# 86885974647565434342125458569795756674/torch.distributed.pipeline.sync.Pipe

Hardware: AMD Instinct MI355X
Metric: tokens/sec for 12-layer Transformer at PP=N (pipeline-parallel training) (higher is better)
Workload: dtype bf16

## Files before the change

### mipipe/csrc/kernels/attention.hip

```cpp
#include "common.h"
#include "kernels.h"

namespace mipipe {

namespace {

typedef __attribute__((ext_vector_type(4))) short s16x4;
typedef __attribute__((ext_vector_type(8))) short s16x8;
typedef __attribute__((address_space(3))) s16x4 lds_s16x4;

constexpr int kRows = 64;
constexpr int kThreads = 256;
constexpr float kLog2e = 1.4426950408889634f;

template <int D>
struct Img {
  static constexpr int kRowBytes = 2 * D;
  static constexpr int kChunks = D / 8;
  static constexpr int kBytes = kRows * kRowBytes;
  __device__ static __forceinline__ int f(int r) {
    if constexpr (kChunks >= 16) return (((r ^ (r >> 2)) & 1) << 1) | ((r & 2) << 1) | (r & 8);
    else if constexpr (kChunks == 8) return ((((r >> 1) ^ (r >> 2)) & 1) << 1) | ((r >> 1) & 4);
    else return (((r & 3) << 2) | ((r >> 2) & 3)) & (kChunks - 1);
  }
// ... 533 lines not shown
        ds[j][r] = pr * (dp - dl[r]);
      }
    }
    scratch_write(scr, ds, lane);
    __builtin_amdgcn_s_waitcnt(0xC07F);
    const bf16x8 s0 = scratch_frag(scr, 0, lane);
    const bf16x8 s1 = scratch_frag(scr, 1, lane);
#pragma unroll
    for (int t2 = 0; t2 < ND; ++t2) {
      dq[t2] = __builtin_amdgcn_mfma_f32_16x16x32_bf16(s0, frag_cols<D>(kimg, 16 * t2, 0, lane), dq[t2], 0, 0, 0);
      dq[t2] = __builtin_amdgcn_mfma_f32_16x16x32_bf16(s1, frag_cols<D>(kimg, 16 * t2, 1, lane), dq[t2], 0, 0, 0);
    }
  }
  bf16_t* dQ = reinterpret_cast<bf16_t*>(a.dq) + boff;
#pragma unroll
  for (int t2 = 0; t2 < ND; ++t2)
#pragma unroll
    for (int r = 0; r < 4; ++r)
      dQ[(int64_t)(qrow0 + r) * a.ld_qkv + 16 * t2 + (lane & 15)] = f2bf(dq[t2][r] * a.scale);
}

template <bool CAUSAL>
__global__ void __launch_bounds__(kThreads, 2) attn_dq_wide_kernel(AttnArgs a) {
  constexpr int D = 64, NS = 2, ND = 4, RB = 2;
  extern __shared__ __attribute__((aligned(16))) char smem[];
  char* kimg = smem;
  char* vimg = smem + Img<D>::kBytes;
  bf16_t* scr_all = reinterpret_cast<bf16_t*>(smem + 2 * Img<D>::kBytes);

  const int tid = threadIdx.x, lane = tid & 63, wave = tid >> 6;
  const int qt = CAUSAL ? (int)gridDim.x - 1 - (int)blockIdx.x : (int)blockIdx.x;
  const int bh = blockIdx.y;
  const int b = bh / a.H, h = bh % a.H;
  const int q0 = qt * kWideRows;
  const int wrow0 = q0 + wave * 32;
  const int64_t boff = (int64_t)b * a.sb_qkv + (int64_t)h * a.sh_qkv;
  const int64_t koff = (int64_t)b * a.sb_qkv + (int64_t)kv_head(a, h) * a.sh_qkv;
  const bf16_t* Q = reinterpret_cast<const bf16_t*>(a.q) + boff;
  const bf16_t* K = reinterpret_cast<const bf16_t*>(a.k) + koff;
  const bf16_t* V = reinterpret_cast<const bf16_t*>(a.v) + koff;
  const bf16_t* dO = reinterpret_cast<const bf16_t*>(a.dout) + (int64_t)b * a.sb_o + (int64_t)h * a.sh_o;

  bf16x8 qf[RB][NS], df[RB][NS];
  float lse2[RB][4], dl[RB][4];
  f32x4 dq[RB][ND];
#pragma unroll
  for (int rb = 0; rb < RB; ++rb) {
    const int myrow = wrow0 + 16 * rb + (lane & 15);
#pragma unroll
    for (int s = 0; s < NS; ++s) {
      qf[rb][s] = frag_global(Q + (int64_t)myrow * a.ld_qkv, s, lane);
      df[rb][s] = frag_global(dO + (int64_t)myrow * a.ld_o, s, lane);
    }
    const int qrow0 = wrow0 + 16 * rb + 4 * (lane >> 4);
#pragma unroll
    for (int r = 0; r < 4; ++r) {
      lse2[rb][r] = a.lse[(int64_t)bh * a.S + qrow0 + r] * kLog2e;
      dl[rb][r] = a.delta[(int64_t)bh * a.S + qrow0 + r];
    }
#pragma unroll
    for (int t = 0; t < ND; ++t) dq[rb][t] = f32x4{0.f, 0.f, 0.f, 0.f};
  }
  const float sl2 = a.scale * kLog2e;
  const float pscale = a.p > 0.f ? 1.f / (1.f - a.p) : 1.f;
  const int ntiles = CAUSAL ? (q0 + kWideRows) / kRows : a.S / kRows;

  TileRegs kr, vr;
  load_tile<D>(K, a.ld_qkv, tid, kr);
  load_tile<D>(V, a.ld_qkv, tid, vr);
  for (int t = 0; t < ntiles; ++t) {
    const int k0 = t * kRows;
    __syncthreads();
    store_tile<D>(kimg, tid, kr);
    store_tile<D>(vimg, tid, vr);
    __syncthreads();
    if (t + 1 < ntiles) {
      load_tile<D>(K + (int64_t)(k0 + kRows) * a.ld_qkv, a.ld_qkv, tid, kr);
      load_tile<D>(V + (int64_t)(k0 + kRows) * a.ld_qkv, a.ld_qkv, tid, vr);
    }
    if (CAUSAL && k0 > wrow0 + 31) continue;
    const bool diag = CAUSAL && k0 + kRows - 1 > wrow0;

    f32x4 sacc[RB][4], pacc[RB][4];
#pragma unroll
    for (int rb = 0; rb < RB; ++rb)
#pragma unroll
      for (int j = 0; j < 4; ++j) sacc[rb][j] = pacc[rb][j] = f32x4{0.f, 0.f, 0.f, 0.f};
#pragma unroll
    for (int s = 0; s < NS; ++s)
#pragma unroll
      for (int j = 0; j < 4; ++j) {
        const bf16x8 kfr = frag_rows<D>(kimg, 16 * j, s, lane);
        const bf16x8 vfr = frag_rows<D>(vimg, 16 * j, s, lane);
#pragma unroll
        for (int rb = 0; rb < RB; ++rb) {
          sacc[rb][j] = __builtin_amdgcn_mfma_f32_16x16x32_bf16(qf[rb][s], kfr, sacc[rb][j], 0, 0, 0);
          pacc[rb][j] = __builtin_amdgcn_mfma_f32_16x16x32_bf16(df[rb][s], vfr, pacc[rb][j], 0, 0, 0);
        }
      }
#pragma unroll
    for (int rb = 0; rb < RB; ++rb) {
      const int qrow0 = wrow0 + 16 * rb + 4 * (lane >> 4);
      float ds[4][4];
#pragma unroll
      for (int j = 0; j < 4; ++j) {
        const int key = k0 + 16 * j + (lane & 15);
        uint32_t w[4] = {0xFFFFFFFFu, 0xFFFFFFFFu, 0xFFFFFFFFu, 0xFFFFFFFFu};
        if (a.p > 0.f) {
          const uint4 mw = attn_mask_words(a, bh, qrow0 >> 2, key);
          w[0] = mw.x; w[1] = mw.y; w[2] = mw.z; w[3] = mw.w;
        }
#pragma unroll
        for (int r = 0; r < 4; ++r) {
          float pr = __builtin_amdgcn_exp2f(sacc[rb][j][r] * sl2 - lse2[rb][r]);
          if (diag && key > qrow0 + r) pr = 0.f;
          float dp = pacc[rb][j][r];
          if (a.p > 0.f) dp = w[r] >= a.threshold ? dp * pscale : 0.f;
          ds[j][r] = pr * (dp - dl[rb][r]);
        }
      }
      scratch_write(scr_all + (wave * RB + rb) * 16 * kScrStride, ds, lane);
    }
    __builtin_amdgcn_s_waitcnt(0xC07F);
    bf16x8 sf[RB][2];
#pragma unroll
    for (int rb = 0; rb < RB; ++rb) {
      const bf16_t* scr = scr_all + (wave * RB + rb) * 16 * kScrStride;
      sf[rb][0] = scratch_frag(scr, 0, lane);
      sf[rb][1] = scratch_frag(scr, 1, lane);
    }
#pragma unroll
    for (int t2 = 0; t2 < ND; ++t2)
#pragma unroll
      for (int s = 0; s < 2; ++s) {
        const bf16x8 kc = frag_cols<D>(kimg, 16 * t2, s, lane);
#pragma unroll
        for (int rb = 0; rb < RB; ++rb)
          dq[rb][t2] = __builtin_amdgcn_mfma_f32_16x16x32_bf16(sf[rb][s], kc, dq[rb][t2], 0, 0, 0);
      }
  }
  bf16_t* dQ = reinterpret_cast<bf16_t*>(a.dq) + boff;
#pragma unroll
  for (int rb = 0; rb < RB; ++rb) {
    const int qrow0 = wrow0 + 16 * rb + 4 * (lane >> 4);
#pragma unroll
    for (int t2 = 0; t2 < ND; ++t2)
#pragma unroll
      for (int r = 0; r < 4; ++r)
        dQ[(int64_t)(qrow0 + r) * a.ld_qkv + 16 * t2 + (lane & 15)] = f2bf(dq[rb][t2][r] * a.scale);
  }
}

template <int D, bool CAUSAL>
__global__ void __launch_bounds__(kThreads, D >= 128 ? 1 : 2) attn_dkdv_kernel(AttnArgs a) {
  extern __shared__ __attribute__((aligned(16))) char smem[];
  char* qimg = smem;
  char* dimg = smem + Img<D>::kBytes;
  bf16_t* scr_all = reinterpret_cast<bf16_t*>(smem + 2 * Img<D>::kBytes);
  float* stats = reinterpret_cast<float*>(smem + 2 * Img<D>::kBytes + 4 * 16 * kScrStride * 2);

  const int tid = threadIdx.x, lane = tid & 63, wave = tid >> 6;
  const int kt = blockIdx.x, bh = blockIdx.y;
  const int b = bh / a.H, h = bh % a.H;
  const int k0 = kt * kRows;
  bf16_t* scr = scr_all + wave * 16 * kScrStride;
  const int64_t boff = (int64_t)b * a.sb_qkv + (int64_t)h * a.sh_qkv;
  const int64_t koff = (int64_t)b * a.sb_qkv + (int64_t)kv_head(a, h) * a.sh_qkv;
  const bf16_t* Q = reinterpret_cast<const bf16_t*>(a.q) + boff;
  const bf16_t* K = reinterpret_cast<const bf16_t*>(a.k) + koff;
  const bf16_t* V = reinterpret_cast<const bf16_t*>(a.v) + koff;
  const bf16_t* dO = reinterpret_cast<const bf16_t*>(a.dout) + (int64_t)b * a.sb_o + (int64_t)h * a.sh_o;

  constexpr int NS = D / 32, ND = D / 16;
  bf16x8 kf[NS], vf[NS];
  const int mykey = k0 + wave * 16 + (lane & 15);
#pragma unroll
  for (int s = 0; s < NS; ++s) {
    kf[s] = frag_global(K + (int64_t)mykey * a.ld_qkv, s, lane);
    vf[s] = frag_global(V + (int64_t)mykey * a.ld_qkv, s, lane);
  }
  const int key0 = k0 + wave * 16 + 4 * (lane >> 4);
  f32x4 dk[ND], dv[ND];
#pragma unroll
  for (int t = 0; t < ND; ++t) dk[t] = dv[t] = f32x4{0.f, 0.f, 0.f, 0.f};
  const float sl2 = a.scale * kLog2e;
  const float pscale = a.p > 0.f ? 1.f / (1.f - a.p) : 1.f;
  const int first = CAUSAL ? kt : 0;
  const int nq = a.S / kRows;

  constexpr bool PF = D <= 128;
  TileRegs qr, dr;
  if constexpr (PF) {
    load_tile<D>(Q + (int64_t)first * kRows * a.ld_qkv, a.ld_qkv, tid, qr);
    load_tile<D>(dO + (int64_t)first * kRows * a.ld_o, a.ld_o, tid, dr);
  }
  for (int t = first; t < nq; ++t) {
    const int q0 = t * kRows;
    __syncthreads();
    if constexpr (PF) {
      store_tile<D>(qimg, tid, qr);
      store_tile<D>(dimg, tid, dr);
    } else {
      stage_tile<D>(Q + (int64_t)q0 * a.ld_qkv, a.ld_qkv, qimg, tid);
      stage_tile<D>(dO + (int64_t)q0 * a.ld_o, a.ld_o, dimg, tid);
    }
    if (tid < 64) {
      stats[tid] = a.lse[(int64_t)bh * a.S + q0 + tid] * kLog2e;
      stats[64 + tid] = a.delta[(int64_t)bh * a.S + q0 + tid];
    }
    __syncthreads();
    if constexpr (PF) if (t + 1 < nq) {
      load_tile<D>(Q + (int64_t)(q0 + kRows) * a.ld_qkv, a.ld_qkv, tid, qr);
      load_tile<D>(dO + (int64_t)(q0 + kRows) * a.ld_o, a.ld_o, tid, dr);
    }
    f32x4 sacc[4], pacc[4];
#pragma unroll
    for (int j = 0; j < 4; ++j) sacc[j] = pacc[j] = f32x4{0.f, 0.f, 0.f, 0.f};
#pragma unroll
    for (int s = 0; s < NS; ++s)
#pragma unroll
      for (int j = 0; j < 4; ++j) {
        sacc[j] = __builtin_amdgcn_mfma_f32_16x16x32_bf16(kf[s], frag_rows<D>(qimg, 16 * j, s, lane), sacc[j], 0, 0, 0);
        pacc[j] = __builtin_amdgcn_mfma_f32_16x16x32_bf16(vf[s], frag_rows<D>(dimg, 16 * j, s, lane), pacc[j], 0, 0, 0);
      }
    float pd[4][4], ds[4][4];
#pragma unroll
    for (int j = 0; j < 4; ++j) {
      const int ql = 16 * j + (lane & 15);
      const int q = q0 + ql;
      const float l2 = stats[ql], dl = stats[64 + ql];
      uint32_t kw0 = 0xFFFFFFFFu, kw1 = 0xFFFFFFFFu, kw2 = 0xFFFFFFFFu, kw3 = 0xFFFFFFFFu;
      if (a.p > 0.f) {
        const int t = lane & 3;
        const uint4 mine = attn_mask_words(a, bh, q >> 2, key0 + t);
        auto word = [&](int i) { return i == 0 ? mine.x : (i == 1 ? mine.y : (i == 2 ? mine.z : mine.w)); };
#pragma unroll
        for (int k = 0; k < 4; ++k) {
          const int src = (lane & ~3) | ((t + k) & 3);
          const uint32_t got = (uint32_t)__shfl((int)word((t - k) & 3), src, 64);
          const int r = (t + k) & 3;
          kw0 = r == 0 ? got : kw0;
          kw1 = r == 1 ? got : kw1;
          kw2 = r == 2 ? got : kw2;
          kw3 = r == 3 ? got : kw3;
        }
      }
#pragma unroll
      for (int r = 0; r < 4; ++r) {
        const int key = key0 + r;
        float pr = __builtin_amdgcn_exp2f(sacc[j][r] * sl2 - l2);
        if (CAUSAL && key > q) pr = 0.f;
        float dp = pacc[j][r];
        float pdrop = pr;
        if (a.p > 0.f) {
          const uint32_t w = r == 0 ? kw0 : (r == 1 ? kw1 : (r == 2 ? kw2 : kw3));
          const bool keep = w >= a.threshold;
          pdrop = keep ? pr * pscale : 0.f;
          dp = keep ? dp * pscale : 0.f;
        }
        pd[j][r] = pdrop;
        ds[j][r] = pr * (dp - dl);
      }
    }
    scratch_write(scr, pd, lane);
    __builtin_amdgcn_s_waitcnt(0xC07F);
    bf16x8 f0 = scratch_frag(scr, 0, lane);
    bf16x8 f1 = scratch_frag(scr, 1, lane);
#pragma unroll
    for (int t2 = 0; t2 < ND; ++t2) {
      dv[t2] = __builtin_amdgcn_mfma_f32_16x16x32_bf16(f0, frag_cols<D>(dimg, 16 * t2, 0, lane), dv[t2], 0, 0, 0);
      dv[t2] = __builtin_amdgcn_mfma_f32_16x16x32_bf16(f1, frag_cols<D>(dimg, 16 * t2, 1, lane), dv[t2], 0, 0, 0);
    }
    __builtin_amdgcn_s_waitcnt(0xC07F);
    scratch_write(scr, ds, lane);
    __builtin_amdgcn_s_waitcnt(0xC07F);
    f0 = scratch_frag(scr, 0, lane);
    f1 = scratch_frag(scr, 1, lane);
#pragma unroll
    for (int t2 = 0; t2 < ND; ++t2) {
      dk[t2] = __builtin_amdgcn_mfma_f32_16x16x32_bf16(f0, frag_cols<D>(qimg, 16 * t2, 0, lane), dk[t2], 0, 0, 0);
      dk[t2] = __builtin_amdgcn_mfma_f32_16x16x32_bf16(f1, frag_cols<D>(qimg, 16 * t2, 1, lane), dk[t2], 0, 0, 0);
    }
  }
  const DkvDst dst = dkv_dst<0>(blockIdx.y);
  bf16_t* dK = dst.dk;
  bf16_t* dV = dst.dv;
#pragma unroll
  for (int t2 = 0; t2 < ND; ++t2)
#pragma unroll
    for (int r = 0; r < 4; ++r) {
      const int64_t o = (int64_t)(key0 + r) * dst.ld + 16 * t2 + (lane & 15);
      dK[o] = f2bf(dk[t2][r] * a.scale);
      dV[o] = f2bf(dv[t2][r]);
    }
}

namespace shortseq {

constexpr int S = 128;
constexpr int kThreads = 512;
constexpr int kChunk = 64;
constexpr int kChunkImg = S * kChunk * 2;
constexpr int kSqImg = S * S * 2;
constexpr int kStageBytes = 3 * kChunkImg;
constexpr int kPOff = 4 * kChunkImg;
constexpr int kDsOff = kPOff + kSqImg;
constexpr int kSmem = kDsOff + kSqImg;
constexpr int kFwdPOff = 2 * kChunkImg;
constexpr int kFwdSmem = kFwdPOff + kSqImg;

__device__ __forceinline__ int coff(int r, int c16) { return Img<64>::off(r, c16); }
__device__ __forceinline__ int soff(int r, int c16) { return Img<128>::off(r, c16); }

__device__ __forceinline__ void load_chunk(const bf16_t* __restrict__ base, int64_t ld, int d0, int tid, uint4& v0,
                                           uint4& v1) {
  const int r = tid >> 3, c = tid & 7;
  v0 = *reinterpret_cast<const uint4*>(base + (int64_t)r * ld + d0 + 8 * c);
  v1 = *reinterpret_cast<const uint4*>(base + (int64_t)(r + 64) * ld + d0 + 8 * c);
}
__device__ __forceinline__ void store_chunk(char* img, int tid, const uint4& v0, const uint4& v1) {
  const int r = tid >> 3, c = tid & 7;
  *reinterpret_cast<uint4*>(img + coff(r, c)) = v0;
  *reinterpret_cast<uint4*>(img + coff(r + 64, c)) = v1;
}

__device__ __forceinline__ bf16x8 crow(const char* img, int rb, int s, int lane) {
  return *reinterpret_cast<const bf16x8*>(img + coff(rb + (lane & 15), 4 * s + (lane >> 4)));
}
__device__ __forceinline__ bf16x8 ccol(const char* img, int db, int s, int lane) {
  const int g = lane >> 4, q = (lane & 15) >> 2, p = lane & 3;
  const int r0 = 32 * s + 8 * g + q;
  const int c8 = (db >> 2) + p;
  const int o0 = coff(r0, c8 >> 1) + 8 * (c8 & 1);
  const int o1 = coff(r0 + 4, c8 >> 1) + 8 * (c8 & 1);
  const s16x4 lo = __builtin_amdgcn_ds_read_tr16_b64_v4i16((lds_s16x4*)(img + o0));
  const s16x4 hi = __builtin_amdgcn_ds_read_tr16_b64_v4i16((lds_s16x4*)(img + o1));
  return __builtin_bit_cast(bf16x8, __builtin_shufflevector(lo, hi, 0, 1, 2, 3, 4, 5, 6, 7));
}
__device__ __forceinline__ bf16x8 srow(const char* img, int rb, int s, int lane) {
  return *reinterpret_cast<const bf16x8*>(img + soff(rb + (lane & 15), 4 * s + (lane >> 4)));
}
__device__ __forceinline__ bf16x8 scol(const char* img, int ib, int s, int lane) {
  const int g = lane >> 4, q = (lane & 15) >> 2, p = lane & 3;
  const int r0 = 32 * s + 8 * g + q;
  const int c8 = (ib >> 2) + p;
  const int o0 = soff(r0, c8 >> 1) + 8 * (c8 & 1);
  const int o1 = soff(r0 + 4, c8 >> 1) + 8 * (c8 & 1);
  const s16x4 lo = __builtin_amdgcn_ds_read_tr16_b64_v4i16((lds_s16x4*)(img + o0));
  const s16x4 hi = __builtin_amdgcn_ds_read_tr16_b64_v4i16((lds_s16x4*)(img + o1));
  return __builtin_bit_cast(bf16x8, __builtin_shufflevector(lo, hi, 0, 1, 2, 3, 4, 5, 6, 7));
}

template <int D, bool CAUSAL>
__global__ void __launch_bounds__(kThreads, 1) attn_bwd_s128_kernel(AttnArgs a) {
  extern __shared__ __attribute__((aligned(16))) char smem[];
  const int tid = threadIdx.x, lane = tid & 63, wave = __builtin_amdgcn_readfirstlane(tid >> 6);
  const int bh = blockIdx.x;
  const int b = bh / a.H, h = bh % a.H;
  const int64_t boff = (int64_t)b * a.sb_qkv + (int64_t)h * a.sh_qkv;
  const int64_t koff = (int64_t)b * a.sb_qkv + (int64_t)kv_head(a, h) * a.sh_qkv;
  const bf16_t* Q = reinterpret_cast<const bf16_t*>(a.q) + boff;
  const bf16_t* K = reinterpret_cast<const bf16_t*>(a.k) + koff;
  const bf16_t* V = reinterpret_cast<const bf16_t*>(a.v) + koff;
  const bf16_t* dO = reinterpret_cast<const bf16_t*>(a.dout) + (int64_t)b * a.sb_o + (int64_t)h * a.sh_o;
  constexpr int NC = D / kChunk;

  f32x4 sacc[8], pacc[8];
#pragma unroll
  for (int j = 0; j < 8; ++j) sacc[j] = pacc[j] = f32x4{0.f, 0.f, 0.f, 0.f};
  const int myrow = wave * 16 + (lane & 15);
  const bf16_t* qrow = Q + (int64_t)myrow * a.ld_qkv;
  const bf16_t* drow = dO + (int64_t)myrow * a.ld_o;

  uint4 k0, k1, v0, v1;
  load_chunk(K, a.ld_qkv, 0, tid, k0, k1);
  load_chunk(V, a.ld_qkv, 0, tid, v0, v1);
  store_chunk(smem, tid, k0, k1);
  store_chunk(smem + kChunkImg, tid, v0, v1);
  __syncthreads();
#pragma unroll 1
  for (int c = 0; c < NC; ++c) {
    const char* kimg = smem + (c & 1) * 2 * kChunkImg;
    const char* vimg = kimg + kChunkImg;
    if (c + 1 < NC) {
      load_chunk(K, a.ld_qkv, (c + 1) * kChunk, tid, k0, k1);
      load_chunk(V, a.ld_qkv, (c + 1) * kChunk, tid, v0, v1);
    }
    bf16x8 qf[2], df[2];
#pragma unroll
    for (int s2 = 0; s2 < 2; ++s2) {
      qf[s2] = frag_global(qrow + c * kChunk, s2, lane);
      df[s2] = frag_global(drow + c * kChunk, s2, lane);
    }
#pragma unroll
    for (int s2 = 0; s2 < 2; ++s2)
#pragma unroll
      for (int j = 0; j < 8; ++j) {
        sacc[j] = __builtin_amdgcn_mfma_f32_16x16x32_bf16(qf[s2], crow(kimg, 16 * j, s2, lane), sacc[j], 0, 0, 0);
        pacc[j] = __builtin_amdgcn_mfma_f32_16x16x32_bf16(df[s2], crow(vimg, 16 * j, s2, lane), pacc[j], 0, 0, 0);
      }
    if (c + 1 < NC) {
      char* nimg = smem + ((c + 1) & 1) * 2 * kChunkImg;
      store_chunk(nimg, tid, k0, k1);
      store_chunk(nimg + kChunkImg, tid, v0, v1);
    }
    __syncthreads();
  }

  const int qrow0 = wave * 16 + 4 * (lane >> 4);
  const float sl2 = a.scale * kLog2e;
  const float pscale = a.p > 0.f ? 1.f / (1.f - a.p) : 1.f;
  float lse2[4];
#pragma unroll
  for (int r = 0; r < 4; ++r) lse2[r] = a.lse[(int64_t)bh * S + qrow0 + r] * kLog2e;
  float dsum[4] = {0.f, 0.f, 0.f, 0.f};
#pragma unroll
  for (int j = 0; j < 8; ++j) {
    const int key = 16 * j + (lane & 15);
    uint32_t w[4] = {0xFFFFFFFFu, 0xFFFFFFFFu, 0xFFFFFFFFu, 0xFFFFFFFFu};
    if (a.p > 0.f) {
      const uint4 mw = attn_mask_words(a, bh, qrow0 >> 2, key);
      w[0] = mw.x; w[1] = mw.y; w[2] = mw.z; w[3] = mw.w;
    }
#pragma unroll
    for (int r = 0; r < 4; ++r) {
      float pr = __builtin_amdgcn_exp2f(sacc[j][r] * sl2 - lse2[r]);
      if (CAUSAL && key > qrow0 + r) pr = 0.f;
      float dp = pacc[j][r];
      float pd = pr;
      if (a.p > 0.f) {
        const bool keep = w[r] >= a.threshold;
        dp = keep ? dp * pscale : 0.f;
        pd = keep ? pr * pscale : 0.f;
      }
      sacc[j][r] = pr;
      pacc[j][r] = dp;
      dsum[r] += pr * dp;
      *reinterpret_cast<bf16_t*>(smem + kPOff + soff(qrow0 + r, key >> 3) + 2 * (key & 7)) = f2bf(pd);
    }
  }
  float delta[4];
#pragma unroll
  for (int r = 0; r < 4; ++r) delta[r] = row_reduce_sum16(dsum[r]);
#pragma unroll
  for (int j = 0; j < 8; ++j) {
    const int key = 16 * j + (lane & 15);
#pragma unroll
    for (int r = 0; r < 4; ++r) {
      const float ds = sacc[j][r] * (pacc[j][r] - delta[r]);
      *reinterpret_cast<bf16_t*>(smem + kDsOff + soff(qrow0 + r, key >> 3) + 2 * (key & 7)) = f2bf(ds);
    }
  }

  const char* pimg = smem + kPOff;
  const char* dsimg = smem + kDsOff;
  char* kimg = smem;
  char* qimg = smem + kChunkImg;
  char* dimg = smem + 2 * kChunkImg;
  const int r0 = wave * 16;
  uint4 a0, a1, b0, b1, e0, e1;
  load_chunk(K, a.ld_qkv, 0, tid, a0, a1);
  load_chunk(Q, a.ld_qkv, 0, tid, b0, b1);
  load_chunk(dO, a.ld_o, 0, tid, e0, e1);
#pragma unroll 1
  for (int c = 0; c < NC; ++c) {
    const int d0 = c * kChunk;
    __syncthreads();
    store_chunk(kimg, tid, a0, a1);
    store_chunk(qimg, tid, b0, b1);
    store_chunk(dimg, tid, e0, e1);
    __syncthreads();
    if (c + 1 < NC) {
      load_chunk(K, a.ld_qkv, d0 + kChunk, tid, a0, a1);
      load_chunk(Q, a.ld_qkv, d0 + kChunk, tid, b0, b1);
      load_chunk(dO, a.ld_o, d0 + kChunk, tid, e0, e1);
    }
    f32x4 dq[4], dk[4], dv[4];
#pragma unroll
    for (int t = 0; t < 4; ++t) dq[t] = dk[t] = dv[t] = f32x4{0.f, 0.f, 0.f, 0.f};
#pragma unroll
    for (int ks = 0; ks < 4; ++ks) {
      const bf16x8 a_dq = srow(dsimg, r0, ks, lane);
      const bf16x8 a_dk = scol(dsimg, r0, ks, lane);
      const bf16x8 a_dv = scol(pimg, r0, ks, lane);
#pragma unroll
      for (int t = 0; t < 4; ++t) {
        dq[t] = __builtin_amdgcn_mfma_f32_16x16x32_bf16(a_dq, ccol(kimg, 16 * t, ks, lane), dq[t], 0, 0, 0);
        dk[t] = __builtin_amdgcn_mfma_f32_16x16x32_bf16(a_dk, ccol(qimg, 16 * t, ks, lane), dk[t], 0, 0, 0);
        dv[t] = __builtin_amdgcn_mfma_f32_16x16x32_bf16(a_dv, ccol(dimg, 16 * t, ks, lane), dv[t], 0, 0, 0);
      }
    }
    const int orow = r0 + 4 * (lane >> 4);
    __syncthreads();
#pragma unroll
    for (int t = 0; t < 4; ++t) {
      const int col = 16 * t + (lane & 15);
#pragma unroll
      for (int r = 0; r < 4; ++r) {
        const int at = coff(orow + r, col >> 3) + 2 * (col & 7);
        *reinterpret_cast<bf16_t*>(kimg + at) = f2bf(dq[t][r] * a.scale);
        *reinterpret_cast<bf16_t*>(qimg + at) = f2bf(dk[t][r] * a.scale);
        *reinterpret_cast<bf16_t*>(dimg + at) = f2bf(dv[t][r]);
      }
    }
    __syncthreads();
    {
      const int r = tid >> 3, cc = tid & 7;
      const DkvDst dst = dkv_dst<0>(blockIdx.x);
      bf16_t* dK = dst.dk;
      bf16_t* dV = dst.dv;
      bf16_t* dQ = dq_dst<0>(blockIdx.x);
#pragma unroll
      for (int h2 = 0; h2 < 2; ++h2) {
        const int row = r + 64 * h2;
        const int off = coff(row, cc);
        const int64_t g = (int64_t)row * a.ld_qkv + d0 + 8 * cc;
        const int64_t gk = (int64_t)row * dst.ld + d0 + 8 * cc;
        *reinterpret_cast<uint4*>(dQ + g) = *reinterpret_cast<const uint4*>(kimg + off);
        *reinterpret_cast<uint4*>(dK + gk) = *reinterpret_cast<const uint4*>(qimg + off);
        *reinterpret_cast<uint4*>(dV + gk) = *reinterpret_cast<const uint4*>(dimg + off);
      }
    }
  }
}

template <int D, bool CAUSAL>
__global__ void __launch_bounds__(kThreads, 2) attn_fwd_s128_kernel(AttnArgs a) {
  extern __shared__ __attribute__((aligned(16))) char smem[];
  const int tid = threadIdx.x, lane = tid & 63, wave = __builtin_amdgcn_readfirstlane(tid >> 6);
  const int bh = blockIdx.x;
  const int b = bh / a.H, h = bh % a.H;
  const int64_t boff = (int64_t)b * a.sb_qkv + (int64_t)h * a.sh_qkv;
  const int64_t koff = (int64_t)b * a.sb_qkv + (int64_t)kv_head(a, h) * a.sh_qkv;
  const bf16_t* Q = reinterpret_cast<const bf16_t*>(a.q) + boff;
  const bf16_t* K = reinterpret_cast<const bf16_t*>(a.k) + koff;
  const bf16_t* V = reinterpret_cast<const bf16_t*>(a.v) + koff;
  constexpr int NC = D / kChunk;

  f32x4 sacc[8];
#pragma unroll
  for (int j = 0; j < 8; ++j) sacc[j] = f32x4{0.f, 0.f, 0.f, 0.f};
  const bf16_t* qrow = Q + (int64_t)(wave * 16 + (lane & 15)) * a.ld_qkv;

  uint4 k0, k1;
  load_chunk(K, a.ld_qkv, 0, tid, k0, k1);
  store_chunk(smem, tid, k0, k1);
  __syncthreads();
#pragma unroll 1
  for (int c = 0; c < NC; ++c) {
    const char* kimg = smem + (c & 1) * kChunkImg;
    if (c + 1 < NC) load_chunk(K, a.ld_qkv, (c + 1) * kChunk, tid, k0, k1);
    bf16x8 qf[2];
#pragma unroll
    for (int s2 = 0; s2 < 2; ++s2) qf[s2] = frag_global(qrow + c * kChunk, s2, lane);
#pragma unroll
    for (int s2 = 0; s2 < 2; ++s2)
#pragma unroll
      for (int j = 0; j < 8; ++j)
        sacc[j] = __builtin_amdgcn_mfma_f32_16x16x32_bf16(qf[s2], crow(kimg, 16 * j, s2, lane), sacc[j], 0, 0, 0);
    if (c + 1 < NC) store_chunk(smem + ((c + 1) & 1) * kChunkImg, tid, k0, k1);
    __syncthreads();
  }

  const int qrow0 = wave * 16 + 4 * (lane >> 4);
  const float sl2 = a.scale * kLog2e;
  const float pscale = a.p > 0.f ? 1.f / (1.f - a.p) : 1.f;
  float mx[4] = {-INFINITY, -INFINITY, -INFINITY, -INFINITY};
#pragma unroll
  for (int j = 0; j < 8; ++j) {
    const int key = 16 * j + (lane & 15);
#pragma unroll
    for (int r = 0; r < 4; ++r) {
      float x = sacc[j][r] * sl2;
      if (CAUSAL && key > qrow0 + r) x = -INFINITY;
      sacc[j][r] = x;
      mx[r] = fmaxf(mx[r], x);
    }
  }
#pragma unroll
  for (int r = 0; r < 4; ++r) mx[r] = row_reduce_max16(mx[r]);
  float sum[4] = {0.f, 0.f, 0.f, 0.f};
#pragma unroll
  for (int j = 0; j < 8; ++j)
#pragma unroll
    for (int r = 0; r < 4; ++r) {
      const float e = __builtin_amdgcn_exp2f(sacc[j][r] - mx[r]);
      sacc[j][r] = e;
      sum[r] += e;
    }
  float inv[4];
#pragma unroll
  for (int r = 0; r < 4; ++r) {
    sum[r] = row_reduce_sum16(sum[r]);
    inv[r] = 1.f / sum[r];
  }
  char* pimg = smem + kFwdPOff;
#pragma unroll
  for (int j = 0; j < 8; ++j) {
    const int key = 16 * j + (lane & 15);
    uint32_t w[4] = {0xFFFFFFFFu, 0xFFFFFFFFu, 0xFFFFFFFFu, 0xFFFFFFFFu};
    if (a.p > 0.f) {
      const uint4 mw = attn_mask_words(a, bh, qrow0 >> 2, key);
      w[0] = mw.x; w[1] = mw.y; w[2] = mw.z; w[3] = mw.w;
    }
#pragma unroll
    for (int r = 0; r < 4; ++r) {
      float pv = sacc[j][r] * inv[r];
      if (a.p > 0.f) pv = w[r] >= a.threshold ? pv * pscale : 0.f;
      *reinterpret_cast<bf16_t*>(pimg + soff(qrow0 + r, key >> 3) + 2 * (key & 7)) = f2bf(pv);
    }
  }
  if ((lane & 15) == 0) {
#pragma unroll
    for (int r = 0; r < 4; ++r) a.lse[(int64_t)bh * S + qrow0 + r] = (mx[r] + log2f(sum[r])) / kLog2e;
  }

  bf16_t* O = reinterpret_cast<bf16_t*>(a.o) + (int64_t)b * a.sb_o + (int64_t)h * a.sh_o;
  uint4 v0, v1;
  load_chunk(V, a.ld_qkv, 0, tid, v0, v1);
  store_chunk(smem, tid, v0, v1);
  __syncthreads();
  const int r0 = wave * 16;
#pragma unroll 1
  for (int c = 0; c < NC; ++c) {
    const char* vimg = smem + (c & 1) * kChunkImg;
    if (c + 1 < NC) load_chunk(V, a.ld_qkv, (c + 1) * kChunk, tid, v0, v1);
    f32x4 o[4];
#pragma unroll
    for (int t = 0; t < 4; ++t) o[t] = f32x4{0.f, 0.f, 0.f, 0.f};
#pragma unroll
    for (int ks = 0; ks < 4; ++ks) {
      const bf16x8 ap = srow(pimg, r0, ks, lane);
#pragma unroll
      for (int t = 0; t < 4; ++t)
        o[t] = __builtin_amdgcn_mfma_f32_16x16x32_bf16(ap, ccol(vimg, 16 * t, ks, lane), o[t], 0, 0, 0);
    }
    const int orow = r0 + 4 * (lane >> 4);
#pragma unroll
    for (int t = 0; t < 4; ++t)
#pragma unroll
      for (int r = 0; r < 4; ++r)
        O[(int64_t)(orow + r) * a.ld_o + c * kChunk + 16 * t + (lane & 15)] = f2bf(o[t][r]);
    if (c + 1 < NC) store_chunk(smem + ((c + 1) & 1) * kChunkImg, tid, v0, v1);
    __syncthreads();
  }
}

}

template <int D>
size_t fwd_smem() { return 2 * Img<D>::kBytes + 4 * 16 * kScrStride * 2; }
template <int D>
size_t dkdv_smem() { return fwd_smem<D>() + 128 * sizeof(float); }

int g_attn_fused_bwd = 1;
const int g_attn_wide = [] {
  const char* e = getenv("MIPIPE_ATTN_WIDE");
  return e == nullptr ? 1 : atoi(e);
}();

template <typename Kern>
void set_smem(Kern k, size_t bytes) {
  hipFuncSetAttribute(reinterpret_cast<const void*>(k), hipFuncAttributeMaxDynamicSharedMemorySize, (int)bytes);
}

template <int D, bool CAUSAL>
void run_fwd(const AttnArgs& a, hipStream_t s) {
  if (a.S == shortseq::S && g_attn_fused_bwd) {
    static bool once_s = false;
    if (!once_s) {
      set_smem(shortseq::attn_fwd_s128_kernel<D, CAUSAL>, shortseq::kFwdSmem);
      once_s = true;
    }
    hipLaunchKernelGGL((shortseq::attn_fwd_s128_kernel<D, CAUSAL>), dim3(a.B * a.H), dim3(shortseq::kThreads),
                       shortseq::kFwdSmem, s, a);
    return;
  }
  if (D == 64 && a.S % kWideRows == 0 && g_attn_wide) {
    static bool once_w = false;
    if (!once_w) { set_smem(attn_fwd_wide_kernel<CAUSAL>, wide_fwd_smem()); once_w = true; }
    hipLaunchKernelGGL((attn_fwd_wide_kernel<CAUSAL>), dim3(a.S / kWideRows, a.B * a.H), dim3(kThreads),
                       wide_fwd_smem(), s, a);
    return;
  }
  const size_t sm = fwd_smem<D>();
  static bool once = false;
  if (!once) { set_smem(attn_fwd_kernel<D, CAUSAL>, sm); once = true; }
  hipLaunchKernelGGL((attn_fwd_kernel<D, CAUSAL>), dim3(a.S / kRows, a.B * a.H), dim3(kThreads), sm, s, a);
}

template <int D, bool CAUSAL>
void run_bwd(const AttnArgs& a, hipStream_t s) {
  const size_t sm = fwd_smem<D>(), sm2 = dkdv_smem<D>();
  static bool once = false;
  if (!once) {
    set_smem(attn_dq_kernel<D, CAUSAL>, sm);
    set_smem(attn_dkdv_kernel<D, CAUSAL>, sm2);
    once = true;
  }
  if (a.S == shortseq::S && g_attn_fused_bwd) {
    static bool once_s = false;
    if (!once_s) {
      set_smem(shortseq::attn_bwd_s128_kernel<D, CAUSAL>, shortseq::kSmem);
      once_s = true;
    }
    hipLaunchKernelGGL((shortseq::attn_bwd_s128_kernel<D, CAUSAL>), dim3(a.B * a.H), dim3(shortseq::kThreads),
                       shortseq::kSmem, s, a);
    return;
  }
  const int64_t rows = (int64_t)a.B * a.S * a.H;
  hipLaunchKernelGGL(attn_delta_kernel, dim3((unsigned)((rows + 3) / 4)), dim3(256), 0, s, a, D);
  hipLaunchKernelGGL((attn_dkdv_kernel<D, CAUSAL>), dim3(a.S / kRows, a.B * a.H), dim3(kThreads), sm2, s, a);
  if (D == 64 && a.S % kWideRows == 0 && g_attn_wide) {
    static bool once_w = false;
    if (!once_w) { set_smem(attn_dq_wide_kernel<CAUSAL>, wide_fwd_smem()); once_w = true; }
    hipLaunchKernelGGL((attn_dq_wide_kernel<CAUSAL>), dim3(a.S / kWideRows, a.B * a.H), dim3(kThreads),
                       wide_fwd_smem(), s, a);
    return;
  }
  hipLaunchKernelGGL((attn_dq_kernel<D, CAUSAL>), dim3(a.S / kRows, a.B * a.H), dim3(kThreads), sm, s, a);
}

}

void attention_set_fused_bwd(int on) { g_attn_fused_bwd = on; }

bool attention_supported(int S, int D) { return S > 0 && S % kRows == 0 && (D == 64 || D == 128 || D == 256); }

void attention_fwd(const AttnArgs& ai, hipStream_t s) {
  AttnArgs a = attn_resolved(ai);
  a.threshold = dropout_threshold(a.p);
  if (a.causal) {
    if (a.D == 64) run_fwd<64, true>(a, s);
    else if (a.D == 128) run_fwd<128, true>(a, s);
    else run_fwd<256, true>(a, s);
  } else {
    if (a.D == 64) run_fwd<64, false>(a, s);
    else if (a.D == 128) run_fwd<128, false>(a, s);
    else run_fwd<256, false>(a, s);
  }
}

void attention_bwd(const AttnArgs& ai, hipStream_t s) {
  AttnArgs a = attn_resolved(ai);
  a.threshold = dropout_threshold(a.p);
  if (a.causal) {
    if (a.D == 64) run_bwd<64, true>(a, s);
    else if (a.D == 128) run_bwd<128, true>(a, s);
    else run_bwd<256, true>(a, s);
  } else {
    if (a.D == 64) run_bwd<64, false>(a, s);
    else if (a.D == 128) run_bwd<128, false>(a, s);
    else run_bwd<256, false>(a, s);
  }
}

}
```

Before: 147,500.

## Keep K resident in LDS and Q/dO fragments in registers for short-seq attention

In the fused S=128 backward kernel, all K chunks now stay resident in LDS and the Q/dO fragments loaded for the score pass are held in registers. The gradient pass reuses them instead of reloading K, Q and dO from global memory, and loads are issued two chunks ahead. The forward kernel prefetches the next Q fragment and the first V chunk during the score loop, and stages the O tile through LDS so global stores are coalesced 16-byte writes. The cost is more registers and LDS, with the full 160KB of LDS used at D=256, which may reduce occupancy.

```diff
diff --git a/mipipe/csrc/kernels/attention.hip b/mipipe/csrc/kernels/attention.hip
--- a/mipipe/csrc/kernels/attention.hip
+++ b/mipipe/csrc/kernels/attention.hip
@@ -859,10 +859,12 @@
 constexpr int kChunk = 64;
 constexpr int kChunkImg = S * kChunk * 2;
 constexpr int kSqImg = S * S * 2;
-constexpr int kStageBytes = 3 * kChunkImg;
-constexpr int kPOff = 4 * kChunkImg;
-constexpr int kDsOff = kPOff + kSqImg;
-constexpr int kSmem = kDsOff + kSqImg;
+constexpr int kBwdVOff = 0;
+constexpr int kBwdPOff = 2 * kChunkImg;
+constexpr int kBwdDsOff = kBwdPOff + kSqImg;
+constexpr int kBwdKOff = kBwdDsOff + kSqImg;
+template <int D> constexpr int bwd_smem() { return kBwdKOff + (D / kChunk) * kChunkImg; }
+static_assert(bwd_smem<256>() == 160 * 1024, "D = 256 uses exactly one CU's LDS");
 constexpr int kFwdPOff = 2 * kChunkImg;
 constexpr int kFwdSmem = kFwdPOff + kSqImg;
 
@@ -892,6 +894,18 @@
   const int o1 = coff(r0 + 4, c8 >> 1) + 8 * (c8 & 1);
   const s16x4 lo = __builtin_amdgcn_ds_read_tr16_b64_v4i16((lds_s16x4*)(img + o0));
   const s16x4 hi = __builtin_amdgcn_ds_read_tr16_b64_v4i16((lds_s16x4*)(img + o1));
+  return __builtin_bit_cast(bf16x8, __builtin_shufflevector(lo, hi, 0, 1, 2, 3, 4, 5, 6, 7));
+}
+__device__ __forceinline__ void ccol_off(int db, int lane, int& o0, int& o1) {
+  const int g = lane >> 4, q = (lane & 15) >> 2, p = lane & 3;
+  const int r0 = 8 * g + q;
+  const int c8 = (db >> 2) + p;
+  o0 = coff(r0, c8 >> 1) + 8 * (c8 & 1);
+  o1 = coff(r0 + 4, c8 >> 1) + 8 * (c8 & 1);
+}
+__device__ __forceinline__ bf16x8 ccol_at(const char* p0, const char* p1, int s) {
+  const s16x4 lo = __builtin_amdgcn_ds_read_tr16_b64_v4i16((lds_s16x4*)(p0 + s * 32 * 2 * kChunk));
+  const s16x4 hi = __builtin_amdgcn_ds_read_tr16_b64_v4i16((lds_s16x4*)(p1 + s * 32 * 2 * kChunk));
   return __builtin_bit_cast(bf16x8, __builtin_shufflevector(lo, hi, 0, 1, 2, 3, 4, 5, 6, 7));
 }
 __device__ __forceinline__ bf16x8 srow(const char* img, int rb, int s, int lane) {
@@ -929,39 +943,72 @@
   const bf16_t* qrow = Q + (int64_t)myrow * a.ld_qkv;
   const bf16_t* drow = dO + (int64_t)myrow * a.ld_o;
 
-  uint4 k0, k1, v0, v1;
-  load_chunk(K, a.ld_qkv, 0, tid, k0, k1);
-  load_chunk(V, a.ld_qkv, 0, tid, v0, v1);
-  store_chunk(smem, tid, k0, k1);
-  store_chunk(smem + kChunkImg, tid, v0, v1);
+  char* const vbuf = smem + kBwdVOff;
+  char* const kbuf = smem + kBwdKOff;
+  uint4 ka0, ka1, va0, va1, kb0, kb1, vb0, vb1;
+  load_chunk(K, a.ld_qkv, 0, tid, ka0, ka1);
+  load_chunk(V, a.ld_qkv, 0, tid, va0, va1);
+
+  bf16x8 qf[NC][2], df[NC][2];
+#pragma unroll
+  for (int s2 = 0; s2 < 2; ++s2) {
+    qf[0][s2] = frag_global(qrow, s2, lane);
+    df[0][s2] = frag_global(drow, s2, lane);
+  }
+  if (NC > 1) {
+    load_chunk(K, a.ld_qkv, kChunk, tid, kb0, kb1);
+    load_chunk(V, a.ld_qkv, kChunk, tid, vb0, vb1);
+  }
+#pragma unroll
+  for (int c = 1; c < NC; ++c)
+#pragma unroll
+    for (int s2 = 0; s2 < 2; ++s2) {
+      qf[c][s2] = frag_global(qrow + c * kChunk, s2, lane);
+      df[c][s2] = frag_global(drow + c * kChunk, s2, lane);
+    }
+  store_chunk(kbuf, tid, ka0, ka1);
+  store_chunk(vbuf, tid, va0, va1);
   __syncthreads();
-#pragma unroll 1
+#pragma unroll
   for (int c = 0; c < NC; ++c) {
-    const char* kimg = smem + (c & 1) * 2 * kChunkImg;
-    const char* vimg = kimg + kChunkImg;
+    const char* kimg = kbuf + c * kChunkImg;
+    const char* vimg = vbuf + (c & 1) * kChunkImg;
+    if (c + 2 < NC) {
+      if (c & 1) {
+        load_chunk(K, a.ld_qkv, (c + 2) * kChunk, tid, kb0, kb1);
+        load_chunk(V, a.ld_qkv, (c + 2) * kChunk, tid, vb0, vb1);
+      } else {
+        load_chunk(K, a.ld_qkv, (c + 2) * kChunk, tid, ka0, ka1);
+        load_chunk(V, a.ld_qkv, (c + 2) * kChunk, tid, va0, va1);
+      }
+    }
+#pragma unroll
+    for (int s2 = 0; s2 < 2; ++s2)
+#pragma unroll
+      for (int j = 0; j < 8; ++j) {
+        sacc[j] = __builtin_amdgcn_mfma_f32_16x16x32_bf16(qf[c][s2], crow(kimg, 16 * j, s2, lane), sacc[j], 0, 0, 0);
+        pacc[j] = __builtin_amdgcn_mfma_f32_16x16x32_bf16(df[c][s2], crow(vimg, 16 * j, s2, lane), pacc[j], 0, 0, 0);
+      }
     if (c + 1 < NC) {
-      load_chunk(K, a.ld_qkv, (c + 1) * kChunk, tid, k0, k1);
-      load_chunk(V, a.ld_qkv, (c + 1) * kChunk, tid, v0, v1);
-    }
-    bf16x8 qf[2], df[2];
-#pragma unroll
-    for (int s2 = 0; s2 < 2; ++s2) {
-      qf[s2] = frag_global(qrow + c * kChunk, s2, lane);
-      df[s2] = frag_global(drow + c * kChunk, s2, lane);
-    }
-#pragma unroll
-    for (int s2 = 0; s2 < 2; ++s2)
-#pragma unroll
-      for (int j = 0; j < 8; ++j) {
-        sacc[j] = __builtin_amdgcn_mfma_f32_16x16x32_bf16(qf[s2], crow(kimg, 16 * j, s2, lane), sacc[j], 0, 0, 0);
-        pacc[j] = __builtin_amdgcn_mfma_f32_16x16x32_bf16(df[s2], crow(vimg, 16 * j, s2, lane), pacc[j], 0, 0, 0);
-      }
-    if (c + 1 < NC) {
-      char* nimg = smem + ((c + 1) & 1) * 2 * kChunkImg;
-      store_chunk(nimg, tid, k0, k1);
-      store_chunk(nimg + kChunkImg, tid, v0, v1);
-    }
-    __syncthreads();
+      char* nk = kbuf + (c + 1) * kChunkImg;
+      char* nv = vbuf + ((c + 1) & 1) * kChunkImg;
+      if ((c + 1) & 1) {
+        store_chunk(nk, tid, kb0, kb1);
+        store_chunk(nv, tid, vb0, vb1);
+      } else {
+        store_chunk(nk, tid, ka0, ka1);
+        store_chunk(nv, tid, va0, va1);
+      }
+    }
+    __syncthreads();
+  }
+  char* const qimg = vbuf;
+  char* const dimg = vbuf + kChunkImg;
+#pragma unroll
+  for (int s2 = 0; s2 < 2; ++s2) {
+    const int at = coff(myrow, 4 * s2 + (lane >> 4));
+    *reinterpret_cast<bf16x8*>(qimg + at) = qf[0][s2];
+    *reinterpret_cast<bf16x8*>(dimg + at) = df[0][s2];
   }
 
   const int qrow0 = wave * 16 + 4 * (lane >> 4);
@@ -993,7 +1040,7 @@
       sacc[j][r] = pr;
       pacc[j][r] = dp;
       dsum[r] += pr * dp;
-      *reinterpret_cast<bf16_t*>(smem + kPOff + soff(qrow0 + r, key >> 3) + 2 * (key & 7)) = f2bf(pd);
+      *reinterpret_cast<bf16_t*>(smem + kBwdPOff + soff(qrow0 + r, key >> 3) + 2 * (key & 7)) = f2bf(pd);
     }
   }
   float delta[4];
@@ -1005,36 +1052,45 @@
 #pragma unroll
     for (int r = 0; r < 4; ++r) {
       const float ds = sacc[j][r] * (pacc[j][r] - delta[r]);
-      *reinterpret_cast<bf16_t*>(smem + kDsOff + soff(qrow0 + r, key >> 3) + 2 * (key & 7)) = f2bf(ds);
-    }
-  }
-
-  const char* pimg = smem + kPOff;
-  const char* dsimg = smem + kDsOff;
-  char* kimg = smem;
-  char* qimg = smem + kChunkImg;
-  char* dimg = smem + 2 * kChunkImg;
+      *reinterpret_cast<bf16_t*>(smem + kBwdDsOff + soff(qrow0 + r, key >> 3) + 2 * (key & 7)) = f2bf(ds);
+    }
+  }
+
+  const char* pimg = smem + kBwdPOff;
+  const char* dsimg = smem + kBwdDsOff;
   const int r0 = wave * 16;
-  uint4 a0, a1, b0, b1, e0, e1;
-  load_chunk(K, a.ld_qkv, 0, tid, a0, a1);
-  load_chunk(Q, a.ld_qkv, 0, tid, b0, b1);
-  load_chunk(dO, a.ld_o, 0, tid, e0, e1);
 #pragma unroll 1
   for (int c = 0; c < NC; ++c) {
     const int d0 = c * kChunk;
-    __syncthreads();
-    store_chunk(kimg, tid, a0, a1);
-    store_chunk(qimg, tid, b0, b1);
-    store_chunk(dimg, tid, e0, e1);
-    __syncthreads();
-    if (c + 1 < NC) {
-      load_chunk(K, a.ld_qkv, d0 + kChunk, tid, a0, a1);
-      load_chunk(Q, a.ld_qkv, d0 + kChunk, tid, b0, b1);
-      load_chunk(dO, a.ld_o, d0 + kChunk, tid, e0, e1);
-    }
+    char* kimg = kbuf + c * kChunkImg;
+    if (NC > 1 && c > 0) {
+      __syncthreads();
+#pragma unroll
+      for (int s2 = 0; s2 < 2; ++s2) {
+        const int at = coff(myrow, 4 * s2 + (lane >> 4));
+        *reinterpret_cast<bf16x8*>(qimg + at) = qf[NC > 1 ? 1 : 0][s2];
+        *reinterpret_cast<bf16x8*>(dimg + at) = df[NC > 1 ? 1 : 0][s2];
+      }
+#pragma unroll
+      for (int i = 1; i + 1 < NC; ++i)
+#pragma unroll
+        for (int s2 = 0; s2 < 2; ++s2) {
+          qf[i][s2] = qf[i + 1][s2];
+          df[i][s2] = df[i + 1][s2];
+        }
+    }
+    __syncthreads();
     f32x4 dq[4], dk[4], dv[4];
 #pragma unroll
     for (int t = 0; t < 4; ++t) dq[t] = dk[t] = dv[t] = f32x4{0.f, 0.f, 0.f, 0.f};
+    const char *kp0[4], *kp1[4];
+#pragma unroll
+    for (int t = 0; t < 4; ++t) {
+      int o0, o1;
+      ccol_off(16 * t, lane, o0, o1);
+      kp0[t] = kimg + o0;
+      kp1[t] = kimg + o1;
+    }
 #pragma unroll
     for (int ks = 0; ks < 4; ++ks) {
       const bf16x8 a_dq = srow(dsimg, r0, ks, lane);
@@ -1042,7 +1098,7 @@
       const bf16x8 a_dv = scol(pimg, r0, ks, lane);
 #pragma unroll
       for (int t = 0; t < 4; ++t) {
-        dq[t] = __builtin_amdgcn_mfma_f32_16x16x32_bf16(a_dq, ccol(kimg, 16 * t, ks, lane), dq[t], 0, 0, 0);
+        dq[t] = __builtin_amdgcn_mfma_f32_16x16x32_bf16(a_dq, ccol_at(kp0[t], kp1[t], ks), dq[t], 0, 0, 0);
         dk[t] = __builtin_amdgcn_mfma_f32_16x16x32_bf16(a_dk, ccol(qimg, 16 * t, ks, lane), dk[t], 0, 0, 0);
         dv[t] = __builtin_amdgcn_mfma_f32_16x16x32_bf16(a_dv, ccol(dimg, 16 * t, ks, lane), dv[t], 0, 0, 0);
       }
@@ -1099,24 +1155,42 @@
   for (int j = 0; j < 8; ++j) sacc[j] = f32x4{0.f, 0.f, 0.f, 0.f};
   const bf16_t* qrow = Q + (int64_t)(wave * 16 + (lane & 15)) * a.ld_qkv;
 
+  constexpr bool kAhead = NC > 1, kStage = NC > 1;
+  constexpr int VB = kAhead ? NC : 0;
+  bf16x8 qf[2], qn[2];
+#pragma unroll
+  for (int s2 = 0; s2 < 2; ++s2) qn[s2] = qf[s2] = frag_global(qrow, s2, lane);
   uint4 k0, k1;
   load_chunk(K, a.ld_qkv, 0, tid, k0, k1);
   store_chunk(smem, tid, k0, k1);
   __syncthreads();
-#pragma unroll 1
+#pragma unroll
   for (int c = 0; c < NC; ++c) {
     const char* kimg = smem + (c & 1) * kChunkImg;
-    if (c + 1 < NC) load_chunk(K, a.ld_qkv, (c + 1) * kChunk, tid, k0, k1);
-    bf16x8 qf[2];
-#pragma unroll
-    for (int s2 = 0; s2 < 2; ++s2) qf[s2] = frag_global(qrow + c * kChunk, s2, lane);
+    if (c + 1 < NC) {
+      load_chunk(K, a.ld_qkv, (c + 1) * kChunk, tid, k0, k1);
+      if (kAhead) {
+#pragma unroll
+        for (int s2 = 0; s2 < 2; ++s2) qn[s2] = frag_global(qrow + (c + 1) * kChunk, s2, lane);
+      }
+    } else if (kAhead) {
+      load_chunk(V, a.ld_qkv, 0, tid, k0, k1);
+    }
+    if (!kAhead && c > 0) {
+#pragma unroll
+      for (int s2 = 0; s2 < 2; ++s2) qf[s2] = frag_global(qrow + c * kChunk, s2, lane);
+    }
 #pragma unroll
     for (int s2 = 0; s2 < 2; ++s2)
 #pragma unroll
       for (int j = 0; j < 8; ++j)
         sacc[j] = __builtin_amdgcn_mfma_f32_16x16x32_bf16(qf[s2], crow(kimg, 16 * j, s2, lane), sacc[j], 0, 0, 0);
-    if (c + 1 < NC) store_chunk(smem + ((c + 1) & 1) * kChunkImg, tid, k0, k1);
-    __syncthreads();
+    if (c + 1 < NC || kAhead) store_chunk(smem + ((c + 1) & 1) * kChunkImg, tid, k0, k1);
+    __syncthreads();
+    if (kAhead) {
+#pragma unroll
+      for (int s2 = 0; s2 < 2; ++s2) qf[s2] = qn[s2];
+    }
   }
 
   const int qrow0 = wave * 16 + 4 * (lane >> 4);
@@ -1173,15 +1247,16 @@
   }
 
   bf16_t* O = reinterpret_cast<bf16_t*>(a.o) + (int64_t)b * a.sb_o + (int64_t)h * a.sh_o;
-  uint4 v0, v1;
-  load_chunk(V, a.ld_qkv, 0, tid, v0, v1);
-  store_chunk(smem, tid, v0, v1);
+  if (!kAhead) {
+    load_chunk(V, a.ld_qkv, 0, tid, k0, k1);
+    store_chunk(smem, tid, k0, k1);
+  }
   __syncthreads();
   const int r0 = wave * 16;
-#pragma unroll 1
+#pragma unroll
   for (int c = 0; c < NC; ++c) {
-    const char* vimg = smem + (c & 1) * kChunkImg;
-    if (c + 1 < NC) load_chunk(V, a.ld_qkv, (c + 1) * kChunk, tid, v0, v1);
+    char* vimg = smem + ((VB + c) & 1) * kChunkImg;
+    if (c + 1 < NC) load_chunk(V, a.ld_qkv, (c + 1) * kChunk, tid, k0, k1);
     f32x4 o[4];
 #pragma unroll
     for (int t = 0; t < 4; ++t) o[t] = f32x4{0.f, 0.f, 0.f, 0.f};
@@ -1193,13 +1268,35 @@
         o[t] = __builtin_amdgcn_mfma_f32_16x16x32_bf16(ap, ccol(vimg, 16 * t, ks, lane), o[t], 0, 0, 0);
     }
     const int orow = r0 + 4 * (lane >> 4);
-#pragma unroll
-    for (int t = 0; t < 4; ++t)
+    if (!kStage) {
+#pragma unroll
+      for (int t = 0; t < 4; ++t)
+#pragma unroll
+        for (int r = 0; r < 4; ++r)
+          O[(int64_t)(orow + r) * a.ld_o + c * kChunk + 16 * t + (lane & 15)] = f2bf(o[t][r]);
+      if (c + 1 < NC) store_chunk(smem + ((VB + c + 1) & 1) * kChunkImg, tid, k0, k1);
+      __syncthreads();
+      continue;
+    }
+    __syncthreads();
+#pragma unroll
+    for (int t = 0; t < 4; ++t) {
+      const int col = 16 * t + (lane & 15);
 #pragma unroll
       for (int r = 0; r < 4; ++r)
-        O[(int64_t)(orow + r) * a.ld_o + c * kChunk + 16 * t + (lane & 15)] = f2bf(o[t][r]);
-    if (c + 1 < NC) store_chunk(smem + ((c + 1) & 1) * kChunkImg, tid, v0, v1);
-    __syncthreads();
+        *reinterpret_cast<bf16_t*>(vimg + coff(orow + r, col >> 3) + 2 * (col & 7)) = f2bf(o[t][r]);
+    }
+    if (c + 1 < NC) store_chunk(smem + ((VB + c + 1) & 1) * kChunkImg, tid, k0, k1);
+    __syncthreads();
+    {
+      const int r = tid >> 3, cc = tid & 7;
+#pragma unroll
+      for (int h2 = 0; h2 < 2; ++h2) {
+        const int row = r + 64 * h2;
+        *reinterpret_cast<uint4*>(O + (int64_t)row * a.ld_o + c * kChunk + 8 * cc) =
+            *reinterpret_cast<const uint4*>(vimg + coff(row, cc));
+      }
+    }
   }
 }
 
@@ -1258,11 +1355,11 @@
   if (a.S == shortseq::S && g_attn_fused_bwd) {
     static bool once_s = false;
     if (!once_s) {
-      set_smem(shortseq::attn_bwd_s128_kernel<D, CAUSAL>, shortseq::kSmem);
+      set_smem(shortseq::attn_bwd_s128_kernel<D, CAUSAL>, shortseq::bwd_smem<D>());
       once_s = true;
     }
     hipLaunchKernelGGL((shortseq::attn_bwd_s128_kernel<D, CAUSAL>), dim3(a.B * a.H), dim3(shortseq::kThreads),
-                       shortseq::kSmem, s, a);
+                       shortseq::bwd_smem<D>(), s, a);
     return;
   }
   const int64_t rows = (int64_t)a.B * a.S * a.H;
```

New measurement: 147,900, median of 6. Within noise of the previous version (+0.2%).
